# Nuralamsiddik16/Ultrafnd_git

Hardware: AMD Instinct MI355X
Metric: train-step samples/sec (FakeSV batch, seq128+224^2) (higher is better)
Workload: dtype bf16

## Files before the change

### ultrafnd_git_amd/csrc/gemm_bf16_kernel.hpp

```cpp
#pragma once

#include <type_traits>

#include "common.hpp"
#include "attn_softmax.hpp"

#pragma clang fp contract(off)

namespace {

constexpr int BK = 64;

struct GemmArgs {
  const __bf16* A;
  const __bf16* W;
  const float* bias;
  const float* residual;
  __bf16* out_bf16;
  float* out_f32;
  int M, N, K, lda, ldw, ldr, ldo, ldf, act;
  int m_tiles, n_tiles;
  unsigned long long* stamps;
  const float* a_stats;
  const float* colsum;
  const float* r_stats;
  const float* r_gamma;
  const float* r_beta;
  float* out_stats;
  int a_parts, r_parts;
  float a_eps, r_eps, inv_h;
  const int32_t* att_mask;
  __bf16* att_ctx;
  int att_h;
  int xcd_cols;
  float att_scale_log2e;
  const __bf16* residual_b;
  int ldrb;
  int ksplit;
  size_t slab_stride;
  const __bf16* aux;
  int ldaux;
  float* guard;
  int pp_rows;
  const int* m_live;
  const int32_t* att_cu;
  const int32_t* att_bins;
  const int* att_nbins;
  int att_t;
};

__device__ __forceinline__ void dma16(const void* gsrc, void* lds_dst) {
  __builtin_amdgcn_global_load_lds((const void __attribute__((address_space(1)))*)gsrc,
                                   (void __attribute__((address_space(3)))*)lds_dst, 16, 0, 0);
}

__device__ __forceinline__ float opaque_f(float x) {
  asm volatile("" : "+v"(x));
  return x;
}
__device__ __forceinline__ f32x2 opaque_f2(f32x2 x) {
  asm volatile("" : "+v"(x));
  return x;
}


__device__ __forceinline__ f32x2 ln_mean_var(const float sm, const float sq, const float inv_h) {
  const float mean = __fmul_rn(sm, inv_h);
  const float var = fmaxf(__fmaf_rn(-mean, mean, __fmul_rn(sq, inv_h)), 0.f);
  return f32x2{mean, var};
}
__device__ __forceinline__ float ln_rstd(const float var, const float eps) {
  return __builtin_amdgcn_rsqf(__fadd_rn(var, eps));
}
__device__ __forceinline__ float ln_guard_ratio(const float mean, const float rstd) {
  const float ratio = __fmul_rn(fabsf(mean), rstd);
  return ratio == ratio ? ratio : INFINITY;
}
template <bool FOLD, int ACT>
__device__ __forceinline__ f32x2 epi_fold_bias_act(f32x2 v, const f32x2 mean2, const f32x2 rstd2, const float cs, const float b) {
  if constexpr (FOLD) v = opaque_f2(rstd2 * __builtin_elementwise_fma(-mean2, f32x2{cs, cs}, v));
  v = v + f32x2{b, b};
  if constexpr (ACT == UFND_ACT_GELU) v = gelu_fast_f2(v);
  else if constexpr (ACT == UFND_ACT_QUICK_GELU) v = quick_gelu_fast_f2(v);
  return v;
}
__device__ __forceinline__ void epi_residual_ln(float (&r)[8], const f32x2 ms, const float (&g8)[8], const float (&b8)[8]) {
#pragma unroll
  for (int q = 0; q < 8; ++q) r[q] = __fmaf_rn(__fmul_rn(__fsub_rn(r[q], ms[0]), ms[1]), g8[q], b8[q]);
}
__device__ __forceinline__ void epi_add8(float (&v)[8], const float (&r)[8]) {
#pragma unroll
  for (int q = 0; q < 8; ++q) v[q] = __fadd_rn(v[q], r[q]);
}
__device__ __forceinline__ f32x2 epi_row_partial(const float (&v)[8]) {
  float sm = 0.f, sq = 0.f;
#pragma unroll
  for (int q = 0; q < 8; ++q) { sm = __fadd_rn(sm, v[q]); sq = __fmaf_rn(v[q], v[q], sq); }
  sm += quad_xor1(sm);
  sq += quad_xor1(sq);
  sm += quad_xor2(sm);
  sq += quad_xor2(sq);
  return f32x2{sm, sq};
}
__device__ __forceinline__ bf16x8 epi_round_bf16x8(const float (&v)[8]) {
  bf16x8 o;
#pragma unroll
  for (int q = 0; q < 8; ++q) o[q] = (__bf16)v[q];
  return o;
}


template <int N>
__device__ __forceinline__ void wait_vmcnt() {
  static_assert(N >= 0 && N <= 63, "vmcnt range");
  asm volatile("s_waitcnt vmcnt(%0)" ::"n"(N) : "memory");
}

template <int V> struct IntC { static constexpr int value = V; };

constexpr int gemm_waves_per_simd(int BM, int BN, int WM, int WN, int STA, int STB, int MI, int LNX, int ATT) {
  const int ring = (STA * BM + STB * BN) * 128, cbytes = WM * WN * MI * (BN / WN + 4) * 4;
  const int smem = (ring > cbytes ? ring : cbytes) + (LNX ? BM * 8 + 64 : 0);
  return (!ATT && smem <= 80 * 1024 ? 2 : 1) * WM * WN / 4;
}
template <int BM, int BN, int WM, int WN, int STA, int STB, int MI, int ABL = 0, int DBG = 0, int LNX = 0, int ATT = 0, int BWD = 0>
__global__ __launch_bounds__(WM * WN * 64) __attribute__((amdgpu_waves_per_eu(gemm_waves_per_simd(BM, BN, WM, WN, STA, STB, MI, LNX, ATT))))
void gemm_bf16_kernel(const GemmArgs a) {
  static_assert(!BWD || (!LNX && !ATT && !ABL && !DBG), "backward forms are plain kernels");
  static_assert(MI == 16 || MI == 32, "MFMA shape");
  static_assert(!ATT || (((BM == 128 && BN == 384 && ATT == 1) || (BM == 256 && BN == 192)) && MI == 16 && WM * WN == 8 && LNX == 1 && ATT <= 2),
                "fused attention tile");
  constexpr bool VIT = ATT == 1 && BM == 256;
  constexpr bool TIL = ATT == 2;
  constexpr bool ONEH = VIT || TIL;
  using acc_t = typename std::conditional<MI == 16, f32x4, f32x16>::type;
  constexpr int AR = MI * MI / 64;
  constexpr int KQ = MI == 16 ? 1 : 2;
  constexpr int NW = WM * WN;
  constexpr int TM = BM / WM, TN = BN / WN;
  constexpr int MT = TM / MI, NT = TN / MI;
  constexpr int ASLOT = BM * 128, BSLOT = BN * 128;
  constexpr int DA = STA - 1, DB = STB - 1;
  constexpr int APIECES = BM / 8, BPIECES = BN / 8;
  constexpr int PWA = APIECES / NW, PWB = (BPIECES + NW - 1) / NW;
  constexpr int WAITN = PWA * (DA - 1 > 0 ? DA - 1 : 0) + PWB * (DB - 1 > 0 ? DB - 1 : 0);
  constexpr int CP = TN + 4;
  constexpr int CBYTES = NW * MI * CP * 4;
  constexpr int RING = STA * ASLOT + STB * BSLOT;
  constexpr int ATT_OFF = (CBYTES + 1023) & ~1023;
  constexpr int ATT_IMG = BM * 128;
  constexpr int ATT_END = ATT ? ATT_OFF + (TIL ? 3 * ATT_IMG + 1024 + 8 * 512 : VIT ? 3 * ATT_IMG + 256 : 6 * ATT_IMG + 2048) : 0;
  constexpr int STAT_OFF0 = (RING > CBYTES) ? RING : CBYTES;
  constexpr int STAT_OFF = STAT_OFF0 > ATT_END ? STAT_OFF0 : ATT_END;
  constexpr int SMEM = STAT_OFF + (LNX ? BM * 8 + 64 : 0);
  static_assert(SMEM <= 160 * 1024, "LDS budget");
  static_assert(APIECES % NW == 0 && TM % MI == 0 && TN % MI == 0, "tile split");
  static_assert(STB >= 2 && (STA == STB || STA == STB + 1), "ring depths");
  static_assert(WAITN <= 63, "vmcnt range");
  __shared__ __attribute__((aligned(16))) char smem[SMEM];

  unsigned long long stamp[10];
  if constexpr (DBG) {
    stamp[0] = __builtin_amdgcn_s_memtime();
    stamp[1] = __builtin_amdgcn_s_memrealtime();
  }

  int mlive = a.M, m_tiles = a.m_tiles;
  if constexpr (!BWD && !ATT) {
    if (a.m_live) {
      const int v = __builtin_amdgcn_readfirstlane(*a.m_live);
      mlive = v < a.M ? (v > 0 ? v : 0) : a.M;
      m_tiles = (mlive + BM - 1) / BM;
      if ((int)blockIdx.x >= m_tiles * a.n_tiles) return;
    }
  }
  if constexpr (ATT) {
    if (a.att_bins) {
      const int v = __builtin_amdgcn_readfirstlane(*a.att_nbins);
      m_tiles = v < a.m_tiles ? (v > 0 ? v : 0) : a.m_tiles;
      if ((int)blockIdx.x >= m_tiles * a.n_tiles) return;
    }
  }
  const int nblk = m_tiles * a.n_tiles;
  int bid, kslice = 0;
  {
    const int ngrid = BWD ? nblk * (a.ksplit > 1 ? a.ksplit : 1) : nblk;
    const int q = ngrid >> 3, r = ngrid & 7, xcd = blockIdx.x & 7, idx = blockIdx.x >> 3;
    bid = (xcd < r ? xcd * (q + 1) : r * (q + 1) + (xcd - r) * q) + idx;
    if constexpr (BWD) {
      kslice = bid / nblk;
      bid -= kslice * nblk;
    }
  }
  int tm = bid / a.n_tiles, tn = bid % a.n_tiles;
  if (a.xcd_cols == 2) {
    const int nh = a.n_tiles >> 1, per_half = m_tiles * nh;
    const int half = bid / per_half, rem = bid - half * per_half;
    tm = rem / nh;
    tn = half * nh + (rem - tm * nh);
  }
  const int m0 = tm * BM, n0 = tn * BN;
  int arow0 = m0, alen = BM;
  int srow[4] = {0, 0, 0, 0}, scnt[4] = {0, 0, 0, 0}, smeta[4] = {-1, -1, -1, -1};
  const bool slots = ATT == 1 && !VIT && a.att_bins != nullptr;
  const int vit_s = VIT ? BM / a.att_t : 0, vit_st = vit_s * a.att_t;
  const int32_t* til = TIL ? a.att_bins + (size_t)tm * UFND_TEXT_TILE_INTS : nullptr;
  int til_rows = 0;
  if constexpr (TIL) til_rows = __builtin_amdgcn_readfirstlane(til[1]);
  if constexpr (VIT) {
    arow0 = tm * vit_st;
    alen = mlive - arow0 < vit_st ? mlive - arow0 : vit_st;
  } else if constexpr (TIL) {
  } else if constexpr (ATT) {
    if (slots) {
      const int32_t* bd = a.att_bins + (size_t)tm * 8;
#pragma unroll
      for (int j = 0; j < 4; ++j) {
        srow[j] = __builtin_amdgcn_readfirstlane(bd[2 * j]);
        smeta[j] = __builtin_amdgcn_readfirstlane(bd[2 * j + 1]);
        const int n = smeta[j] & 255, rest = n - 32 * ((smeta[j] >> 8) & 3);
        scnt[j] = smeta[j] < 0 ? 0 : (rest < 32 ? rest : 32);
      }
#pragma unroll
      for (int j = 1; j < 4; ++j) srow[j] = scnt[j] > 0 ? srow[j] : srow[0];
    } else if (a.att_cu) {
      mlive = __builtin_amdgcn_readfirstlane(*a.m_live);
      arow0 = __builtin_amdgcn_readfirstlane(a.att_cu[tm]);
      alen = __builtin_amdgcn_readfirstlane(a.att_cu[tm + 1]) - arow0;
      if (alen <= 0) return;
    }
  } else {
    alen = mlive - m0;
  }
  auto tile_row = [&](int tr) {
    if constexpr (TIL) return (int)til[UFND_TEXT_TILE_ROWMAP + tr];
    if (slots) {
      const int j = tr >> 5, q = tr & 31;
      const int r0 = j == 0 ? srow[0] : j == 1 ? srow[1] : j == 2 ? srow[2] : srow[3];
      const int c = j == 0 ? scnt[0] : j == 1 ? scnt[1] : j == 2 ? scnt[2] : scnt[3];
      return r0 + (q < c ? q : (c > 0 ? c - 1 : 0));
    }
    const int gr = arow0 + tr;
    return gr < mlive ? gr : mlive - 1;
  };
  auto tile_row_live = [&](int tr) {
    if constexpr (TIL) return tr < til_rows;
    if (slots) {
      const int j = tr >> 5;
      return (tr & 31) < (j == 0 ? scnt[0] : j == 1 ? scnt[1] : j == 2 ? scnt[2] : scnt[3]);
    }
    return tr < alen;
  };
  const int wave = __builtin_amdgcn_readfirstlane(threadIdx.x >> 6), lane = threadIdx.x & 63;
  const int wm = wave / WN, wn = wave % WN, fr = lane & (MI - 1), g = lane / MI;

  acc_t acc[MT][NT];
#pragma unroll
  for (int i = 0; i < MT; ++i)
#pragma unroll
    for (int j = 0; j < NT; ++j)
#pragma unroll
      for (int r = 0; r < AR; ++r) acc[i][j][r] = 0.f;

  int nk = a.K / BK, kbase = 0;
  if constexpr (BWD) {
    if (a.ksplit > 1) {
      const int per = (nk + a.ksplit - 1) / a.ksplit;
      kbase = kslice * per * BK;
      nk = nk - kslice * per < per ? nk - kslice * per : per;
    }
  }
  const int prow = lane >> 3, ppos = lane & 7;
  int arow_att[ATT ? PWA : 1];
  if constexpr (ATT) {
#pragma unroll
    for (int ii = 0; ii < PWA; ++ii) arow_att[ii] = tile_row(8 * (wave + NW * ii) + prow);
  }
  auto issueA = [&](int t, int kt) {
    char* buf = smem + (t % STA) * ASLOT;
    const int k0 = kbase + kt * BK;
#pragma unroll
    for (int ii = 0; ii < PWA; ++ii) {
      const int p = wave + NW * ii;
      const int r = 8 * p + prow;
      const int c = ppos ^ ((r >> 1) & 7);
      int gr = arow0 + r;
      gr = gr < mlive ? gr : mlive - 1;
      if constexpr (ATT) gr = arow_att[ii];
      dma16(a.A + (size_t)gr * a.lda + k0 + c * 8, buf + p * 1024);
    }
  };
  auto issueB = [&](int t, int kt) {
    char* buf = smem + STA * ASLOT + (t % STB) * BSLOT;
    const int k0 = kbase + kt * BK;
#pragma unroll
    for (int ii = 0; ii < PWB; ++ii) {
      int p = wave + NW * ii;
      if constexpr (BPIECES % NW != 0) p = p < BPIECES ? p : p - BPIECES;
      const int r = 8 * p + prow;
      const int c = ppos ^ ((r >> 1) & 7);
      int gr = n0 + r;
      gr = gr < a.N ? gr : a.N - 1;
      if constexpr (ONEH) gr = (r >> 6) * a.att_h + tn * 64 + (r & 63);
      else if constexpr (ATT) gr = (r >> 7) * a.att_h + tn * 128 + (r & 127);
      dma16(a.W + (size_t)gr * a.ldw + k0 + c * 8, buf + p * 1024);
    }
  };
  constexpr int TPR = NW * 64 / BM;
  static_assert(!LNX || TPR == 2 || TPR == 4, "threads per tile row");
  constexpr int GPT = 4 / (TPR < 4 ? TPR : 4);
  f32x4 sv[GPT][3];
  f32x2* st_lds = reinterpret_cast<f32x2*>(smem + STAT_OFF);
  const float* sp = nullptr;
  if constexpr (LNX) {
    sp = a.a_stats ? a.a_stats : a.r_stats;
    if (sp) {
      const int parts = a.a_stats ? a.a_parts : a.r_parts;
      int row = arow0 + (int)threadIdx.x / TPR;
      row = row < mlive ? row : mlive - 1;
      if constexpr (ATT) row = tile_row((int)threadIdx.x / TPR);
      const f32x4* base = reinterpret_cast<const f32x4*>(sp + (size_t)row * parts * 2);
      const int nq = parts >> 1, sub = threadIdx.x % TPR;
#pragma unroll
      for (int gi = 0; gi < GPT; ++gi)
#pragma unroll
        for (int u = 0; u < 3; ++u) {
          const int q = (sub + gi * TPR) + 4 * u;
          asm volatile("global_load_dwordx4 %0, %1, off" : "=v"(sv[gi][u]) : "v"(base + (q < nq ? q : 0)) : "memory");
        }
    }
  }
  float til_kb = 0.0f;
  if constexpr (TIL) {
    if (threadIdx.x < BM) til_kb = __int_as_float(til[UFND_TEXT_TILE_KBIAS + threadIdx.x]);
  }
  int att_mk = 1;
  if constexpr (ATT == 1 && !VIT) {
    if (slots) {
      const int j = (int)threadIdx.x >> 7, k = threadIdx.x & 127;
      const int mt = j == 0 ? smeta[0] : j == 1 ? smeta[1] : j == 2 ? smeta[2] : smeta[3];
      att_mk = mt >= 0 && k < (mt & 255);
      if (att_mk && a.att_mask) att_mk = a.att_mask[(size_t)(mt >> 10) * BM + k];
    } else if (a.att_mask && threadIdx.x < BM) {
      att_mk = a.att_mask[m0 + threadIdx.x];
    }
  }
#pragma unroll
  for (int s = 0; s < STA; ++s) {
    const int ks = s < nk ? s : nk - 1;
    if (s < STB && (LNX || s < nk)) issueB(s, ks);
    if (LNX || s < nk) issueA(s, ks);
  }

  if constexpr (LNX) {
    if (sp) {
      constexpr int NPRO = STA * PWA + STB * PWB;
      static_assert(NPRO <= 63, "vmcnt range");
      if constexpr (GPT == 1)
        asm volatile("s_waitcnt vmcnt(%3) ; STATRETIRE %0 %1 %2" : "+v"(sv[0][0]), "+v"(sv[0][1]), "+v"(sv[0][2]) : "n"(NPRO) : "memory");
      else
        asm volatile("s_waitcnt vmcnt(%6) ; STATRETIRE %0 %1 %2 %3 %4 %5" : "+v"(sv[0][0]), "+v"(sv[0][1]), "+v"(sv[0][2]), "+v"(sv[GPT - 1][0]),
                     "+v"(sv[GPT - 1][1]), "+v"(sv[GPT - 1][2]) : "n"(NPRO) : "memory");
      const int nq_ = (a.a_stats ? a.a_parts : a.r_parts) >> 1, sub_ = threadIdx.x % TPR;
      float gs[GPT], gq[GPT];
#pragma unroll
      for (int gi = 0; gi < GPT; ++gi) {
#pragma unroll
        for (int u = 0; u < 3; ++u) {
          if ((sub_ + gi * TPR) + 4 * u >= nq_) sv[gi][u] = f32x4{0.f, 0.f, 0.f, 0.f};
        }
        gs[gi] = sv[gi][0][0] + sv[gi][0][2];
        gq[gi] = sv[gi][0][1] + sv[gi][0][3];
#pragma unroll
        for (int u = 1; u < 3; ++u) { gs[gi] += sv[gi][u][0] + sv[gi][u][2]; gq[gi] += sv[gi][u][1] + sv[gi][u][3]; }
      }
      float sm, sq;
      if constexpr (TPR == 4) {
        sm = gs[0] + quad_xor1(gs[0]);
        sq = gq[0] + quad_xor1(gq[0]);
        sm += quad_xor2(sm);
        sq += quad_xor2(sq);
      } else {
        const float s01 = gs[0] + quad_xor1(gs[0]), s23 = gs[1] + quad_xor1(gs[1]);
        const float q01 = gq[0] + quad_xor1(gq[0]), q23 = gq[1] + quad_xor1(gq[1]);
        sm = s01 + s23;
        sq = q01 + q23;
      }
      const f32x2 mv = ln_mean_var(sm, sq, a.inv_h);
      const f32x2 ms = {mv[0], ln_rstd(mv[1], a.a_stats ? a.a_eps : a.r_eps)};
      if (threadIdx.x % TPR == 0) st_lds[threadIdx.x / TPR] = ms;
      if (a.guard && a.a_stats) {
        const float ratio = ln_guard_ratio(ms[0], ms[1]);
        const float worst = wave_max(threadIdx.x % TPR == 0 && tile_row_live((int)threadIdx.x / TPR) ? ratio : 0.0f);
        if (lane == 0) reinterpret_cast<float*>(smem + STAT_OFF + BM * 8)[wave] = worst;
      }
      asm volatile("s_waitcnt lgkmcnt(0)" ::: "memory");
    }
  }

  bf16x8 af0[KQ][MT], bf0[KQ][NT], af1[KQ][MT], bf1[KQ][NT];
  auto read_half = [&](int t, auto kk_, bf16x8 (&af)[KQ][MT], bf16x8 (&bfr)[KQ][NT]) {
    constexpr int kk = decltype(kk_)::value;
    const char* At = smem + (t % STA) * ASLOT;
    const char* Bt = smem + STA * ASLOT + (t % STB) * BSLOT;
#pragma unroll
    for (int q = 0; q < KQ; ++q) {
      const int chunk = MI == 16 ? g + 4 * kk : g + 2 * q + 4 * kk;
#pragma unroll
      for (int i = 0; i < MT; ++i) af[q][i] = lds_frag(At, wm * TM + i * MI + fr, chunk);
#pragma unroll
      for (int j = 0; j < NT; ++j) bfr[q][j] = lds_frag(Bt, wn * TN + j * MI + fr, chunk);
    }
  };
  auto mma_half = [&](const bf16x8 (&af)[KQ][MT], const bf16x8 (&bfr)[KQ][NT]) {
#pragma unroll
    for (int q = 0; q < KQ; ++q)
#pragma unroll
      for (int i = 0; i < MT; ++i)
#pragma unroll
        for (int j = 0; j < NT; ++j) {
          if constexpr (MI == 16) acc[i][j] = __builtin_amdgcn_mfma_f32_16x16x32_bf16(af[q][i], bfr[q][j], acc[i][j], 0, 0, 0);
          else acc[i][j] = __builtin_amdgcn_mfma_f32_32x32x16_bf16(af[q][i], bfr[q][j], acc[i][j], 0, 0, 0);
        }
  };
  constexpr int NMF = KQ * MT * NT, NRD = KQ * (MT + NT);
  auto body = [&](int t, auto ia_, auto ib_, auto next_) {
    constexpr bool IA = decltype(ia_)::value != 0, IB = decltype(ib_)::value != 0, NEXT = decltype(next_)::value != 0;
    if constexpr (ABL != 1) {
      read_half(t, IntC<1>{}, af1, bf1);
      mma_half(af0, bf0);
#pragma unroll
      for (int q = 0; q < (NRD < NMF ? NRD : NMF - 1); ++q) {
        __builtin_amdgcn_sched_group_barrier(0x008, 1, 0);
        __builtin_amdgcn_sched_group_barrier(0x100, 1, 0);
      }
      __builtin_amdgcn_sched_group_barrier(0x100, NRD - (NRD < NMF ? NRD : NMF - 1), 0);
      __builtin_amdgcn_sched_group_barrier(0x008, NMF - (NRD < NMF ? NRD : NMF - 1), 0);
    }
    if constexpr (NEXT) {
      __builtin_amdgcn_sched_barrier(0);
      if (t + STA - 1 < nk) wait_vmcnt<WAITN>();
      else wait_vmcnt<0>();
      asm volatile("s_waitcnt lgkmcnt(0)" ::: "memory");
      __builtin_amdgcn_s_barrier();
      __builtin_amdgcn_sched_barrier(0);
      if constexpr (ABL != 1) read_half(t + 1, IntC<0>{}, af0, bf0);
      if constexpr (ABL != 2) {
        if constexpr (IB) issueB(t + STB, t + STB);
        if constexpr (IA) issueA(t + STA, t + STA);
      }
    }
    if constexpr (ABL != 1) {
      mma_half(af1, bf1);
      constexpr int PW = (ABL == 2 || !NEXT) ? 0 : (IA ? PWA : 0) + (IB ? PWB : 0);
      constexpr int GRP = (NMF - 1) / (PW + 1) > 0 ? (NMF - 1) / (PW + 1) : 1;
      if constexpr (NEXT && NRD + PW < NMF) {
#pragma unroll
        for (int q = 0; q < NRD; ++q) {
          __builtin_amdgcn_sched_group_barrier(0x008, 1, 0);
          __builtin_amdgcn_sched_group_barrier(0x100, 1, 0);
        }
        constexpr int REST = NMF - NRD, G2 = REST / (PW + 1) > 0 ? REST / (PW + 1) : 1;
#pragma unroll
        for (int q = 0; q < PW; ++q) {
          __builtin_amdgcn_sched_group_barrier(0x008, G2, 0);
          __builtin_amdgcn_sched_group_barrier(0x020, 1, 0);
        }
        __builtin_amdgcn_sched_group_barrier(0x008, REST - G2 * PW > 0 ? REST - G2 * PW : 0, 0);
      } else {
        __builtin_amdgcn_sched_group_barrier(0x008, 1, 0);
        if constexpr (NEXT) __builtin_amdgcn_sched_group_barrier(0x100, NRD, 0);
#pragma unroll
        for (int q = 0; q < PW; ++q) {
          __builtin_amdgcn_sched_group_barrier(0x008, GRP, 0);
          __builtin_amdgcn_sched_group_barrier(0x020, 1, 0);
        }
        __builtin_amdgcn_sched_group_barrier(0x008, NMF - 1 - GRP * PW > 0 ? NMF - 1 - GRP * PW : 0, 0);
      }
    }
  };

  if (STA <= nk) wait_vmcnt<PWA * (STA - 1) + PWB * (STB - 1)>();
  else wait_vmcnt<0>();
  __builtin_amdgcn_sched_barrier(0);
  __builtin_amdgcn_s_barrier();
  __builtin_amdgcn_sched_barrier(0);
  if constexpr (DBG) {
    stamp[2] = __builtin_amdgcn_s_memtime();
    stamp[3] = __builtin_amdgcn_s_memrealtime();
  }
  if constexpr (ABL != 1) read_half(0, IntC<0>{}, af0, bf0);
  int t = 0;
  for (; t + STA < nk; ++t) body(t, IntC<1>{}, IntC<1>{}, IntC<1>{});
  for (; t + STB < nk; ++t) body(t, IntC<0>{}, IntC<1>{}, IntC<1>{});
  for (; t + 1 < nk; ++t) body(t, IntC<0>{}, IntC<0>{}, IntC<1>{});
  body(t, IntC<0>{}, IntC<0>{}, IntC<0>{});
  __builtin_amdgcn_sched_barrier(0);
  __builtin_amdgcn_s_barrier();
  __builtin_amdgcn_sched_barrier(0);
  if constexpr (DBG) {
    stamp[4] = __builtin_amdgcn_s_memtime();
    stamp[5] = __builtin_amdgcn_s_memrealtime();
  }

  float bj[NT], csj[NT];
#pragma unroll
  for (int j = 0; j < NT; ++j) { bj[j] = 0.f; csj[j] = 0.f; }
  auto gcol = [&](int c) { return ONEH ? (c >> 6) * a.att_h + tn * 64 + (c & 63) : ATT ? (c >> 7) * a.att_h + tn * 128 + (c & 127) : n0 + c; };
  if (a.bias) {
#pragma unroll
    for (int j = 0; j < NT; ++j) bj[j] = a.bias[gcol(wn * TN + j * MI + fr)];
  }
  bool fold = false, rln = false;
  if constexpr (LNX) {
    fold = a.a_stats != nullptr;
    rln = a.r_stats != nullptr;
    if (fold) {
#pragma unroll
      for (int j = 0; j < NT; ++j) csj[j] = a.colsum[gcol(wn * TN + j * MI + fr)];
    }
  }
  float* cst = reinterpret_cast<float*>(smem) + wave * MI * CP;
  float* const outf = (BWD && a.out_f32) ? a.out_f32 + (size_t)kslice * a.slab_stride : a.out_f32;
  constexpr int CPR = TN / 8;
  constexpr int CHUNKS = MI * CPR;
  constexpr int NIT = (CHUNKS + 63) / 64;
  constexpr bool FIXCOL = (64 % CPR) == 0;
  auto ld8 = [&](const float* ptr, float (&o)[8]) {
    const f32x4 x0 = *reinterpret_cast<const f32x4*>(ptr), x1 = *reinterpret_cast<const f32x4*>(ptr + 4);
#pragma unroll
    for (int q = 0; q < 4; ++q) { o[q] = x0[q]; o[4 + q] = x1[q]; }
  };
  float g8[8], b8[8];
  if constexpr (LNX && FIXCOL) {
    if (rln) {
      const int col = n0 + wn * TN + (lane % CPR) * 8;
      ld8(a.r_gamma + col, g8);
      ld8(a.r_beta + col, b8);
    }
  }
  auto epilogue = [&](auto act_, auto mode_) {
    constexpr int ACT = decltype(act_)::value;
    constexpr bool FOLD = LNX && decltype(mode_)::value == 1, RLN = LNX && decltype(mode_)::value == 2;
    constexpr bool RES = !FOLD;
#pragma unroll
    for (int i = 0; i < MT; ++i) {
      float rr8[RES ? NIT : 1][8];
      if constexpr (RES) if (a.residual && !(BWD && a.aux)) {
#pragma unroll
        for (int it = 0; it < NIT; ++it) {
          const int id = lane + 64 * it;
          if (id < CHUNKS) {
            int row = m0 + wm * TM + i * MI + id / CPR;
            row = row < a.M ? row : a.M - 1;
            ld8(a.residual + (size_t)row * a.ldr + n0 + wn * TN + (id % CPR) * 8, rr8[it]);
          }
        }
      }
      if constexpr (BWD) {
        if (a.aux) {
#pragma unroll
          for (int it = 0; it < NIT; ++it) {
            const int id = lane + 64 * it;
            if (id < CHUNKS) {
              int row = m0 + wm * TM + i * MI + id / CPR;
              row = row < a.M ? row : a.M - 1;
              const bf16x8 xb = *reinterpret_cast<const bf16x8*>(a.aux + (size_t)row * a.ldaux + n0 + wn * TN + (id % CPR) * 8);
#pragma unroll
              for (int q = 0; q < 8; ++q) rr8[it][q] = (float)xb[q];
            }
          }
        }
      }
      if constexpr (LNX && RES) {
        if (a.residual_b) {
#pragma unroll
          for (int it = 0; it < NIT; ++it) {
            const int id = lane + 64 * it;
            if (id < CHUNKS) {
              int row = m0 + wm * TM + i * MI + id / CPR;
              row = row < a.M ? row : a.M - 1;
              const bf16x8 rb = *reinterpret_cast<const bf16x8*>(a.residual_b + (size_t)row * a.ldrb + n0 + wn * TN + (id % CPR) * 8);
#pragma unroll
              for (int q = 0; q < 8; ++q) rr8[it][q] = (float)rb[q];
            }
          }
        }
      }
#pragma unroll
      for (int r = 0; r < AR; r += 2) {
        const int prow_ = MI == 16 ? 4 * g + r : 8 * (r >> 2) + 4 * g + (r & 3);
        f32x2 mean2 = {0.f, 0.f}, rstd2 = {1.f, 1.f};
        if constexpr (FOLD) {
          const f32x2 a0 = st_lds[wm * TM + i * MI + prow_], a1 = st_lds[wm * TM + i * MI + prow_ + 1];
          mean2 = f32x2{a0[0], a1[0]};
          rstd2 = f32x2{a0[1], a1[1]};
        }
#pragma unroll
        for (int j = 0; j < NT; ++j) {
          const f32x2 v = epi_fold_bias_act<FOLD, ACT>(f32x2{acc[i][j][r], acc[i][j][r + 1]}, mean2, rstd2, csj[j], bj[j]);
          cst[prow_ * CP + j * MI + fr] = v.x;
          cst[(prow_ + 1) * CP + j * MI + fr] = v.y;
        }
      }
      asm volatile("s_waitcnt lgkmcnt(0)" ::: "memory");
#pragma unroll
      for (int it = 0; it < NIT; ++it) {
        const int id = lane + 64 * it;
        if (id >= CHUNKS) break;
        const int rr = id / CPR, cl = (id % CPR) * 8;
        const int row = m0 + wm * TM + i * MI + rr;
        const int col = n0 + wn * TN + cl;
        const bool live = row < mlive;
        const f32x4 v0 = *reinterpret_cast<const f32x4*>(cst + rr * CP + cl);
        const f32x4 v1 = *reinterpret_cast<const f32x4*>(cst + rr * CP + cl + 4);
        float v[8] = {v0[0], v0[1], v0[2], v0[3], v1[0], v1[1], v1[2], v1[3]};
        if constexpr (BWD) {
          if (a.aux) {
            if (a.act == UFND_ACT_GELU_BWD) {
#pragma unroll
              for (int q = 0; q < 8; ++q) v[q] = v[q] * gelu_grad_f(rr8[it][q]);
            } else {
#pragma unroll
              for (int q = 0; q < 8; ++q) v[q] = v[q] * quick_gelu_grad_f(rr8[it][q]);
            }
          }
        }
        if constexpr (RES) if ((a.residual && !(BWD && a.aux)) || (LNX && a.residual_b)) {
          if constexpr (RLN) {
            const f32x2 ms = st_lds[wm * TM + i * MI + rr];
            if constexpr (!FIXCOL) {
              ld8(a.r_gamma + col, g8);
              ld8(a.r_beta + col, b8);
            }
            epi_residual_ln(rr8[it], ms, g8, b8);
          }
          epi_add8(v, rr8[it]);
        }
        if constexpr (LNX && RES) {
          if (a.out_stats) {
            if constexpr (CPR % 4 == 0) {
              const f32x2 part = epi_row_partial(v);
              if (live && (id & 3) == 0) *reinterpret_cast<f32x2*>(a.out_stats + ((size_t)row * (a.N >> 5) + (col >> 5)) * 2) = part;
            }
          }
        }
        if constexpr (ATT) {
          const int ct = wn * TN + cl;
          const int trow = wm * TM + i * MI + rr, img = ct >> 6, ch = (ct & 63) >> 3;
          const bf16x8 o = epi_round_bf16x8(v);
          const int sw = img >= (ONEH ? 2 : 4) ? (ch ^ (((trow >> 1) & 3) << 1)) : (ch ^ ((trow >> 1) & 7));
          *reinterpret_cast<bf16x8*>(smem + ATT_OFF + img * ATT_IMG + trow * 128 + (sw << 4)) = o;
          continue;
        }
        if (!live) continue;
        if (a.out_f32) {
          float* op = outf + (size_t)row * a.ldf + col;
          *reinterpret_cast<f32x4*>(op) = f32x4{v[0], v[1], v[2], v[3]};
          *reinterpret_cast<f32x4*>(op + 4) = f32x4{v[4], v[5], v[6], v[7]};
        }
        if (a.out_bf16) *reinterpret_cast<bf16x8*>(a.out_bf16 + (size_t)row * a.ldo + col) = epi_round_bf16x8(v);
      }
      asm volatile("s_waitcnt lgkmcnt(0)" ::: "memory");
    }
  };
  if constexpr (LNX) {
    if (fold) {
      if (a.act == UFND_ACT_GELU) epilogue(IntC<UFND_ACT_GELU>{}, IntC<1>{});
      else if (a.act == UFND_ACT_QUICK_GELU) epilogue(IntC<UFND_ACT_QUICK_GELU>{}, IntC<1>{});
      else epilogue(IntC<UFND_ACT_NONE>{}, IntC<1>{});
    } else if (rln) {
      epilogue(IntC<UFND_ACT_NONE>{}, IntC<2>{});
    } else {
      epilogue(IntC<UFND_ACT_NONE>{}, IntC<0>{});
    }
  } else {
    if (a.act == UFND_ACT_GELU) epilogue(IntC<UFND_ACT_GELU>{}, IntC<0>{});
    else if (a.act == UFND_ACT_QUICK_GELU) epilogue(IntC<UFND_ACT_QUICK_GELU>{}, IntC<0>{});
    else epilogue(IntC<UFND_ACT_NONE>{}, IntC<0>{});
  }
  if constexpr (ATT && DBG) {
    stamp[8] = __builtin_amdgcn_s_memtime();
    stamp[9] = __builtin_amdgcn_s_memrealtime();
  }
  if constexpr (VIT) {
    const int T = a.att_t;
    float* kbias = reinterpret_cast<float*>(smem + ATT_OFF + 3 * ATT_IMG);
    if (threadIdx.x < 64) kbias[threadIdx.x] = (int)threadIdx.x < T ? 0.0f : -INFINITY;
    __syncthreads();
    const int nqb = (T + 31) >> 5, nsamp = alen > 0 ? alen / T : 0;
    for (int u = wave; u < nsamp * nqb; u += NW) {
      const int smp = u / nqb, q0 = (u - smp * nqb) * 32, r0 = smp * T;
      const auto row = [&](int k) { return r0 + (k < T ? k : T - 1); };
      attn_unit<1, false>(smem + ATT_OFF, smem + ATT_OFF + ATT_IMG, smem + ATT_OFF + 2 * ATT_IMG, [&](int q) { return row(q0 + q); }, row, kbias,
                          a.att_scale_log2e, lane, a.att_ctx + (size_t)(arow0 + r0 + q0) * a.att_h + tn * 64, a.att_h, T - q0);
    }
  } else if constexpr (TIL) {
    constexpr float NEG_MASK = -3.0e38f;
    float* kbias = reinterpret_cast<float*>(smem + ATT_OFF + 3 * ATT_IMG);
    float* wbias = kbias + BM + wave * 128;
    if (threadIdx.x < BM) kbias[threadIdx.x] = til_kb;
    __syncthreads();
    int nunits = __builtin_amdgcn_readfirstlane(til[2]);
    nunits = nunits < UFND_TEXT_TILE_UNITS ? nunits : UFND_TEXT_TILE_UNITS;
    for (int u = wave; u < nunits; u += NW) {
      const int unit = __builtin_amdgcn_readfirstlane(til[UFND_TEXT_TILE_UNIT0 + u]);
      const int sj = unit & (UFND_TEXT_TILE_SAMPLES - 1), q0 = ((unit >> 8) & 3) * 32;
      const int grow0 = __builtin_amdgcn_readfirstlane(til[4 + 2 * sj]);
      const int meta = __builtin_amdgcn_readfirstlane(til[5 + 2 * sj]);
      const int r0 = (meta >> 8) & 255;
      int n = meta & 255;
      n = n < 1 ? 1 : (n < BM - r0 ? n : BM - r0);
      n = n < 128 ? n : 128;
#pragma unroll
      for (int h = 0; h < 2; ++h) {
        const int k = lane + 64 * h;
        wbias[k] = k < n ? kbias[r0 + k] : NEG_MASK;
      }
      asm volatile("s_waitcnt lgkmcnt(0)" ::: "memory");
      const auto row = [&](int k) { return r0 + (k < n ? k : n - 1); };
      attn_unit<2, true>(smem + ATT_OFF, smem + ATT_OFF + ATT_IMG, smem + ATT_OFF + 2 * ATT_IMG, [&](int q) { return row(q0 + q); }, row, wbias,
                         a.att_scale_log2e, lane, a.att_ctx + (size_t)(grow0 + q0) * a.att_h + tn * 64, a.att_h, n - q0);
    }
  } else if constexpr (ATT) {
    constexpr float NEG_MASK = -3.0e38f;
    float* kbias = reinterpret_cast<float*>(smem + ATT_OFF + 6 * 16384);
    if (slots || threadIdx.x < BM) kbias[threadIdx.x] = att_mk != 0 ? 0.0f : NEG_MASK;
    __syncthreads();
    const int hh = wave >> 2, wq = wave & 3;
    int wrow0 = arow0 + 32 * wq, wcnt = alen - 32 * wq, koff = 0;
    const float* wbias = kbias;
    if (slots) {
      const int mt = wq == 0 ? smeta[0] : wq == 1 ? smeta[1] : wq == 2 ? smeta[2] : smeta[3];
      wrow0 = wq == 0 ? srow[0] : wq == 1 ? srow[1] : wq == 2 ? srow[2] : srow[3];
      wcnt = wq == 0 ? scnt[0] : wq == 1 ? scnt[1] : wq == 2 ? scnt[2] : scnt[3];
      koff = 32 * (wq - ((mt >> 8) & 3));
      wbias = kbias + wq * BM;
    }
    if (wcnt > 0)
      attn_unit<2, true>(smem + ATT_OFF + hh * 16384, smem + ATT_OFF + (2 + hh) * 16384, smem + ATT_OFF + (4 + hh) * 16384, [&](int q) { return wq * 32 + q; },
                         [&](int k) { return (koff + k) & (BM - 1); }, wbias, a.att_scale_log2e, lane,
                         a.att_ctx + (size_t)wrow0 * a.att_h + (tn * 2 + hh) * 64, a.att_h, wcnt);
  }
  if constexpr (LNX) {
    if (a.guard && a.a_stats && threadIdx.x == 0) {
      const float* gw = reinterpret_cast<const float*>(smem + STAT_OFF + BM * 8);
      float worst = gw[0];
#pragma unroll
      for (int w = 1; w < NW; ++w) worst = fmaxf(worst, gw[w]);
      atomicMax(reinterpret_cast<int*>(a.guard + (blockIdx.x & 1023)), __float_as_int(worst));
    }
  }
  if constexpr (DBG) {
    asm volatile("s_waitcnt vmcnt(0)" ::: "memory");
    stamp[6] = __builtin_amdgcn_s_memtime();
    stamp[7] = __builtin_amdgcn_s_memrealtime();
    if (threadIdx.x == 0) {
      constexpr int NS = ATT ? 10 : 8;
#pragma unroll
      for (int i = 0; i < NS; ++i) a.stamps[(size_t)blockIdx.x * NS + i] = stamp[i];
    }
  }
}

}

#define UFND_GEMM_TILES(X)                                                                             \
  X(0, 128, 128, 2, 2, 3, 3, 16, 0, 0)                                                              \
  X(1, 128, 64, 2, 2, 3, 3, 16, 0, 0)                                                 \
  X(2, 256, 128, 4, 2, 3, 3, 16, 1, 1)                                                              \
  X(3, 128, 128, 2, 2, 2, 2, 16, 1, 0)                                                \
  X(4, 128, 64, 2, 2, 4, 4, 16, 0, 0)                                                               \
  X(5, 256, 64, 4, 2, 3, 3, 16, 0, 0)                                                               \
  X(6, 128, 288, 2, 2, 3, 3, 16, 0, 0)                                   \
  X(7, 128, 96, 2, 2, 3, 3, 16, 0, 0)                                     \
  X(8, 256, 192, 4, 2, 2, 2, 16, 1, 1)                                  \
  X(9, 128, 384, 2, 2, 2, 2, 16, 0, 0)                                                              \
  X(10, 128, 192, 2, 2, 3, 3, 16, 0, 0)                                                             \
  X(11, 128, 96, 2, 2, 4, 4, 16, 0, 0)                                                              \
  X(12, 64, 96, 1, 2, 4, 4, 16, 0, 0)                     \
  X(13, 64, 192, 1, 2, 3, 3, 16, 0, 0)                                                              \
  X(14, 128, 256, 2, 2, 2, 2, 16, 0, 0)                                                             \
  X(15, 256, 256, 4, 2, 2, 2, 16, 1, 1)                                                             \
  X(16, 128, 128, 4, 2, 3, 3, 16, 1, 1)                                  \
  X(17, 128, 192, 4, 2, 3, 3, 16, 1, 1)                                  \
  X(18, 256, 64, 4, 2, 4, 4, 16, 0, 0)                                                              \
  X(19, 64, 64, 1, 2, 4, 4, 16, 0, 0)                                                 \
  X(20, 128, 64, 4, 2, 4, 4, 16, 1, 1)                                   \
  X(21, 256, 192, 2, 4, 2, 2, 16, 0, 0)                                          \
  X(22, 256, 192, 4, 2, 3, 2, 16, 1, 1)                                 \
  X(23, 256, 256, 4, 2, 3, 2, 16, 0, 0)                                                             \
  X(24, 128, 192, 4, 2, 4, 4, 16, 0, 0)                                                             \
  X(25, 128, 256, 4, 2, 3, 3, 16, 0, 0)                                 \
  X(26, 256, 192, 4, 2, 2, 2, 32, 0, 0)   \
  X(27, 128, 128, 4, 2, 3, 3, 32, 0, 0)                                                                    \
  X(28, 256, 144, 8, 1, 2, 2, 16, 1, 1)   \
  X(29, 128, 128, 4, 2, 2, 2, 16, 1, 0)   \
  X(30, 256, 128, 4, 2, 3, 2, 16, 1, 0)

#ifdef UFND_DIAG
#define UFND_TILE_BUILT(PROD_) 1
#else
#define UFND_TILE_BUILT(PROD_) (PROD_)
#endif

struct TileCfg { int bm, bn, threads, wn, lnx, built, sta, stb, prod; };
static const TileCfg kTiles[] = {
#define X(id, BM_, BN_, WM_, WN_, SA_, SB_, MI_, LN_, PROD_) {BM_, BN_, WM_ * WN_ * 64, WN_, LN_, UFND_TILE_BUILT(PROD_), SA_, SB_, PROD_},
    UFND_GEMM_TILES(X)
#undef X
};
constexpr int kNumTiles = sizeof(kTiles) / sizeof(kTiles[0]);
constexpr bool gemm_bwd_tile(int id) { return id == 15 || id == 16 || id == 17 || id == 20 || id == 22; }

static int xcd_cols_for(int M, int N, int K, int m_tiles, int n_tiles) {
#ifdef UFND_DIAG
  static const int forced = [] { const char* e = getenv("UFND_GEMM_XCD_COLS"); return e ? atoi(e) : 0; }();
  if (forced == 1) return 1;
  if (forced == 2) return (n_tiles % 2 == 0) ? 2 : 1;
#endif
  (void)K;
  return (4LL * N > (long long)M && n_tiles % 2 == 0 && m_tiles >= 4) ? 2 : 1;
}

static int launch_cfg(int cfg, int mode, GemmArgs& a, hipStream_t stream) {
  if (cfg < 0 || cfg >= kNumTiles || !kTiles[cfg].built) {
    ufnd_set_error("gemm_bf16: tile config %d is not part of this library", cfg);
    return UFND_ERR_INVALID;
  }
  const TileCfg& t = kTiles[cfg];
  a.m_tiles = ufnd_cdiv(a.M, t.bm);
  a.n_tiles = a.N / t.bn;
  a.xcd_cols = xcd_cols_for(a.M, a.N, a.K, a.m_tiles, a.n_tiles);
  const dim3 grid(a.m_tiles * a.n_tiles * (mode == 6 && a.ksplit > 1 ? a.ksplit : 1)), block(t.threads);
#ifdef UFND_GEMM_ONLY_BWD
#define X(id, BM_, BN_, WM_, WN_, SA_, SB_, MI_, LN_, PROD_)                                                                      \
  case id:                                                                                                                        \
    if constexpr (gemm_bwd_tile(id)) {                                                                                            \
      hipLaunchKernelGGL((gemm_bf16_kernel<BM_, BN_, WM_, WN_, SA_, SB_, MI_, 0, 0, 0, 0, 1>), grid, block, 0, stream, a);        \
    } else {                                                                                                                      \
      ufnd_set_error("gemm_bf16 backward: tile %d has no backward kernel", id);                                                   \
      return UFND_ERR_INVALID;                                                                                                    \
    }                                                                                                                             \
    break;
  (void)mode;
  switch (cfg) {
    UFND_GEMM_TILES(X)
    default: ufnd_set_error("gemm_bf16: unknown tile config %d", cfg); return UFND_ERR_INVALID;
  }
#undef X
  return UFND_OK;
#else
#ifdef UFND_DIAG
#define UFND_DIAG_LAUNCH(BM_, BN_, WM_, WN_, SA_, SB_, MI_)                                                                             \
  else if (mode == 5) hipLaunchKernelGGL((gemm_bf16_kernel<BM_, BN_, WM_, WN_, SA_, SB_, MI_, 0, 1, 1>), grid, block, 0, stream, a);   \
  else if (mode == 1) hipLaunchKernelGGL((gemm_bf16_kernel<BM_, BN_, WM_, WN_, SA_, SB_, MI_, 1, 0>), grid, block, 0, stream, a);      \
  else if (mode == 2) hipLaunchKernelGGL((gemm_bf16_kernel<BM_, BN_, WM_, WN_, SA_, SB_, MI_, 2, 0>), grid, block, 0, stream, a);      \
  else if (mode == 3) hipLaunchKernelGGL((gemm_bf16_kernel<BM_, BN_, WM_, WN_, SA_, SB_, MI_, 0, 1>), grid, block, 0, stream, a);
#else
#define UFND_DIAG_LAUNCH(BM_, BN_, WM_, WN_, SA_, SB_, MI_)
#endif
#define X(id, BM_, BN_, WM_, WN_, SA_, SB_, MI_, LN_, PROD_)                                                        \
  case id:                                                                                                          \
    if constexpr (UFND_TILE_BUILT(PROD_) != 0) {                                                                    \
      if (mode == 0) {                                                                                              \
        hipLaunchKernelGGL((gemm_bf16_kernel<BM_, BN_, WM_, WN_, SA_, SB_, MI_, 0, 0>), grid, block, 0, stream, a); \
      } else if constexpr (LN_ != 0) {    \
        if (mode == 4) hipLaunchKernelGGL((gemm_bf16_kernel<BM_, BN_, WM_, WN_, SA_, SB_, MI_, 0, 0, 1>), grid, block, 0, stream, a); \
        UFND_DIAG_LAUNCH(BM_, BN_, WM_, WN_, SA_, SB_, MI_)                                                         \
        else {                                                                                                      \
          ufnd_set_error("gemm_bf16: tile %d has no kernel for mode %d in this library", id, mode);                 \
          return UFND_ERR_INVALID;                                                                                  \
        }                                                                                                           \
      } else {                                                                                                      \
        ufnd_set_error("gemm_bf16: tile %d has no diagnostics / LayerNorm-aware build", id);                        \
        return UFND_ERR_INVALID;                                                                                    \
      }                                                                                                             \
    }                                                                                                               \
    break;
  switch (cfg) {
    UFND_GEMM_TILES(X)
    default: ufnd_set_error("gemm_bf16: unknown tile config %d", cfg); return UFND_ERR_INVALID;
  }
#undef X
#undef UFND_DIAG_LAUNCH
  return UFND_OK;
#endif
}

static int auto_cfg(int M, int N, int K) {
#ifdef UFND_DIAG
  static const int forced = [] { const char* e = getenv("UFND_GEMM_FORCE_CFG"); return e ? atoi(e) : -1; }();
  if (forced >= 0 && forced < kNumTiles && N % kTiles[forced].bn == 0) return forced;
#endif
  auto tiles = [&](int cfg) { return (long long)ufnd_cdiv(M, kTiles[cfg].bm) * (N / kTiles[cfg].bn); };
  if (N % 256 == 0 && N >= 3072 && tiles(15) >= 512) return 15;
  if (N % 256 == 0 && N >= 2048 && tiles(15) >= 190 && tiles(15) <= 256) return 15;
  if (N % 192 == 0 && tiles(22) >= 160) return 22;
  if (N >= 2048) {
    if (N % 192 == 0 && N >= 3072) return 17;
    if (N % 128 == 0) return 16;
  }
  if (N < 2048 && N % 192 == 0 && tiles(17) >= 150 && tiles(17) <= 256) return 17;
  if (N % 128 == 0 && tiles(16) >= 150) return 16;
  return 20;
}
```

Before: 31260.

## Prefetch epilogue residual/aux tiles ahead of use with register-budgeted depth

Restructures the GEMM epilogue so residual, aux and bf16 residual loads for later MT row-tiles are issued one or more iterations before they are consumed. The prefetch depth is chosen at compile time from an estimated VGPR budget, with a rolling per-chunk mode when two full sets do not fit. bf16 sources are kept packed in registers and widened only at use. The aim is to hide global-load latency in the epilogue, at the cost of higher register pressure and possible spills or lower occupancy.

```diff
diff --git a/ultrafnd_git_amd/csrc/gemm_bf16_kernel.hpp b/ultrafnd_git_amd/csrc/gemm_bf16_kernel.hpp
--- a/ultrafnd_git_amd/csrc/gemm_bf16_kernel.hpp
+++ b/ultrafnd_git_amd/csrc/gemm_bf16_kernel.hpp
@@ -92,6 +92,15 @@
 #pragma unroll
   for (int q = 0; q < 8; ++q) v[q] = __fadd_rn(v[q], r[q]);
 }
+__device__ __forceinline__ void epi_keep_bf16x8(float (&r)[8], const f32x4 raw) {
+#pragma unroll
+  for (int q = 0; q < 4; ++q) r[q] = raw[q];
+}
+__device__ __forceinline__ void epi_widen_bf16x8(float (&r)[8]) {
+  const bf16x8 x = __builtin_bit_cast(bf16x8, f32x4{r[0], r[1], r[2], r[3]});
+#pragma unroll
+  for (int q = 0; q < 8; ++q) r[q] = (float)x[q];
+}
 __device__ __forceinline__ f32x2 epi_row_partial(const float (&v)[8]) {
   float sm = 0.f, sq = 0.f;
 #pragma unroll
@@ -122,6 +131,19 @@
   const int ring = (STA * BM + STB * BN) * 128, cbytes = WM * WN * MI * (BN / WN + 4) * 4;
   const int smem = (ring > cbytes ? ring : cbytes) + (LNX ? BM * 8 + 64 : 0);
   return (!ATT && smem <= 80 * 1024 ? 2 : 1) * WM * WN / 4;
+}
+constexpr bool gemm_residual_fits(int sets, int mt, int nt, int ar, int nit, int extra, int waves_per_simd) {
+  const int budget = waves_per_simd > 2 ? 512 / waves_per_simd : 256;
+  return mt * nt * ar + sets * nit * 8 + 32 + 2 * nt + 4 * nit + extra <= budget;
+}
+constexpr int gemm_residual_depth(int mt, int nt, int ar, int nit, int extra, int waves_per_simd, int att) {
+  if (att) return 0;
+  int d = mt;
+  while (d > 1 && !gemm_residual_fits(d < mt ? d + 1 : mt, mt, nt, ar, nit, extra, waves_per_simd)) --d;
+  return d;
+}
+constexpr bool gemm_residual_rolls(int mt, int nt, int ar, int nit, int extra, int waves_per_simd, int att) {
+  return !att && mt > 1 && !gemm_residual_fits(2, mt, nt, ar, nit, extra, waves_per_simd);
 }
 template <int BM, int BN, int WM, int WN, int STA, int STB, int MI, int ABL = 0, int DBG = 0, int LNX = 0, int ATT = 0, int BWD = 0>
 __global__ __launch_bounds__(WM * WN * 64) __attribute__((amdgpu_waves_per_eu(gemm_waves_per_simd(BM, BN, WM, WN, STA, STB, MI, LNX, ATT))))
@@ -543,31 +565,40 @@
     constexpr int ACT = decltype(act_)::value;
     constexpr bool FOLD = LNX && decltype(mode_)::value == 1, RLN = LNX && decltype(mode_)::value == 2;
     constexpr bool RES = !FOLD;
-#pragma unroll
-    for (int i = 0; i < MT; ++i) {
-      float rr8[RES ? NIT : 1][8];
+    constexpr int WPS = gemm_waves_per_simd(BM, BN, WM, WN, STA, STB, MI, LNX, ATT);
+    constexpr int XTRA = (LNX && FIXCOL ? 16 : 0) + (BWD ? 8 : 0);
+    constexpr int DEPTH = RES ? gemm_residual_depth(MT, NT, AR, NIT, XTRA, WPS, ATT) : 0;
+    constexpr bool ROLL = RES && gemm_residual_rolls(MT, NT, AR, NIT, XTRA, WPS, ATT);
+    constexpr int SETS = ROLL ? 1 : DEPTH < MT ? DEPTH + 1 : MT;
+    float rr8[RES ? SETS : 1][RES ? NIT : 1][8];
+    auto request = [&](const int i, const int it0, const int it1) {
       if constexpr (RES) if (a.residual && !(BWD && a.aux)) {
 #pragma unroll
-        for (int it = 0; it < NIT; ++it) {
+        for (int it = it0; it < it1; ++it) {
           const int id = lane + 64 * it;
           if (id < CHUNKS) {
             int row = m0 + wm * TM + i * MI + id / CPR;
             row = row < a.M ? row : a.M - 1;
-            ld8(a.residual + (size_t)row * a.ldr + n0 + wn * TN + (id % CPR) * 8, rr8[it]);
+            ld8(a.residual + (size_t)row * a.ldr + n0 + wn * TN + (id % CPR) * 8, rr8[i % SETS][it]);
           }
         }
       }
       if constexpr (BWD) {
         if (a.aux) {
 #pragma unroll
-          for (int it = 0; it < NIT; ++it) {
+          for (int it = it0; it < it1; ++it) {
             const int id = lane + 64 * it;
             if (id < CHUNKS) {
               int row = m0 + wm * TM + i * MI + id / CPR;
               row = row < a.M ? row : a.M - 1;
-              const bf16x8 xb = *reinterpret_cast<const bf16x8*>(a.aux + (size_t)row * a.ldaux + n0 + wn * TN + (id % CPR) * 8);
-#pragma unroll
-              for (int q = 0; q < 8; ++q) rr8[it][q] = (float)xb[q];
+              const __bf16* src = a.aux + (size_t)row * a.ldaux + n0 + wn * TN + (id % CPR) * 8;
+              if constexpr (DEPTH > 0) {
+                epi_keep_bf16x8(rr8[i % SETS][it], *reinterpret_cast<const f32x4*>(src));
+              } else {
+                const bf16x8 xb = *reinterpret_cast<const bf16x8*>(src);
+#pragma unroll
+                for (int q = 0; q < 8; ++q) rr8[i % SETS][it][q] = (float)xb[q];
+              }
             }
           }
         }
@@ -575,18 +606,29 @@
       if constexpr (LNX && RES) {
         if (a.residual_b) {
 #pragma unroll
-          for (int it = 0; it < NIT; ++it) {
+          for (int it = it0; it < it1; ++it) {
             const int id = lane + 64 * it;
             if (id < CHUNKS) {
               int row = m0 + wm * TM + i * MI + id / CPR;
               row = row < a.M ? row : a.M - 1;
-              const bf16x8 rb = *reinterpret_cast<const bf16x8*>(a.residual_b + (size_t)row * a.ldrb + n0 + wn * TN + (id % CPR) * 8);
-#pragma unroll
-              for (int q = 0; q < 8; ++q) rr8[it][q] = (float)rb[q];
+              const __bf16* src = a.residual_b + (size_t)row * a.ldrb + n0 + wn * TN + (id % CPR) * 8;
+              if constexpr (DEPTH > 0) {
+                epi_keep_bf16x8(rr8[i % SETS][it], *reinterpret_cast<const f32x4*>(src));
+              } else {
+                const bf16x8 rb = *reinterpret_cast<const bf16x8*>(src);
+#pragma unroll
+                for (int q = 0; q < 8; ++q) rr8[i % SETS][it][q] = (float)rb[q];
+              }
             }
           }
         }
       }
+    };
+#pragma unroll
+    for (int i = 0; i < DEPTH; ++i) request(i, 0, NIT);
+#pragma unroll
+    for (int i = 0; i < MT; ++i) {
+      if (!ROLL && (i + DEPTH < MT || DEPTH == 0)) request(i + DEPTH, 0, NIT);
 #pragma unroll
       for (int r = 0; r < AR; r += 2) {
         const int prow_ = MI == 16 ? 4 * g + r : 8 * (r >> 2) + 4 * g + (r & 3);
@@ -617,26 +659,29 @@
         float v[8] = {v0[0], v0[1], v0[2], v0[3], v1[0], v1[1], v1[2], v1[3]};
         if constexpr (BWD) {
           if (a.aux) {
+            if constexpr (DEPTH > 0) epi_widen_bf16x8(rr8[i % SETS][it]);
             if (a.act == UFND_ACT_GELU_BWD) {
 #pragma unroll
-              for (int q = 0; q < 8; ++q) v[q] = v[q] * gelu_grad_f(rr8[it][q]);
+              for (int q = 0; q < 8; ++q) v[q] = v[q] * gelu_grad_f(rr8[i % SETS][it][q]);
             } else {
 #pragma unroll
-              for (int q = 0; q < 8; ++q) v[q] = v[q] * quick_gelu_grad_f(rr8[it][q]);
+              for (int q = 0; q < 8; ++q) v[q] = v[q] * quick_gelu_grad_f(rr8[i % SETS][it][q]);
             }
           }
         }
         if constexpr (RES) if ((a.residual && !(BWD && a.aux)) || (LNX && a.residual_b)) {
+          if constexpr (LNX && DEPTH > 0) if (a.residual_b) epi_widen_bf16x8(rr8[i % SETS][it]);
           if constexpr (RLN) {
             const f32x2 ms = st_lds[wm * TM + i * MI + rr];
             if constexpr (!FIXCOL) {
               ld8(a.r_gamma + col, g8);
               ld8(a.r_beta + col, b8);
             }
-            epi_residual_ln(rr8[it], ms, g8, b8);
+            epi_residual_ln(rr8[i % SETS][it], ms, g8, b8);
           }
-          epi_add8(v, rr8[it]);
-        }
+          epi_add8(v, rr8[i % SETS][it]);
+        }
+        if constexpr (ROLL) if (i + 1 < MT) request(i + 1, it, it + 1);
         if constexpr (LNX && RES) {
           if (a.out_stats) {
             if constexpr (CPR % 4 == 0) {
```

Result: no change. 31150 (-0.4%).
